# ibrahimhroob/SPS

Hardware: AMD Instinct MI355X
Metric: scans/sec @100k pts, 0.1 m voxel (higher is better)
Workload: dtype f32; 1 GPU; BASELINE config 2: single ~100k-pt LiDAR-like scan + variant-B submap, 0.1 m voxel, CustomMinkUNet14 fp32, 1 scan per step per GPU (4 distinct scans cycled); scan_points=100824, rows=153557, streams_per_gpu=8, compact_arenas=True

## Files before the change

### sps_amd/csrc/conv_kernels.inc.h

```cpp

typedef float floatx4 __attribute__((ext_vector_type(4)));

struct ConvArgs {
  const float *in;
  float *out;
  const float *Wu;
  const float *scale;
  const float *shift;
  const float *res;
  const int *nbr;
  const uint32_t *tmask;
  const int *n_out;
  const int *abort_flag;
  int out_rows;
  int64_t ldn;
  int ldi, ldo, ldr;
  int K, cin, cout, NT, upk;
  int relu, S;
  float inv_upk;
  float in_const;
  uint32_t in_bytes, wu_bytes, nbr_bytes;
  int tile_cap;
  int trace_on;
  const float *in2;
  int ldi2, upk2;
  uint32_t in2_bytes;
  const float *fin_w;
  float *fin_out;
  float fin_b;
  const uint32_t *rb_e;
  const unsigned char *rb_k;
  const int *rb_cnt;
  int rb_supertiles;
  const int4 *px_order;
  const int4 *tile_order;
  int order_ways;
  const float *up_Wu, *up_scale, *up_shift;
  const int *up_down;
  const uint32_t *up_tmask;
  float *up_out;
  int64_t up_ldn;
  int up_ldo, up_cout, up_rows;
  uint32_t up_wu_bytes;
};

#ifndef SPS_KCHUNK
#define SPS_KCHUNK 32
#endif
constexpr int KCHUNK = SPS_KCHUNK;
constexpr uint32_t OOR = 0xFFFF0000u;
typedef unsigned int u32x4 __attribute__((ext_vector_type(4)));

#if defined(SPS_WAVE_TRACE)
__device__ unsigned long long g_wave_trace[4 * 32768];
#endif

template <int NTW, int G, int MINW, bool DS, bool FIN, int S, int CG = 1, int UNT = 0, bool U4 = false>
__global__ __launch_bounds__((S == 8 ? 512 : 256) * CG, MINW) void k_conv(ConvArgs a) {
#if defined(SPS_WAVE_TRACE)
  const unsigned long long tr_t0 = wall_clock64();
  unsigned long long tr_t1 = 0;
  int tr_tiles = 0, tr_units = 0;
#endif
  static_assert(CG == 1 || (S == 4 && !FIN), "column groups share a workgroup only in the four-split geometry");
  static_assert(UNT == 0 || S == 4, "the fused transposed convolution needs one tile per workgroup");
  constexpr int NW1 = S == 8 ? 8 : 4;
  constexpr int NWV = NW1 * CG;
  __shared__ unsigned char klist[NWV][128];
  __shared__ uint32_t aoff_s[NWV][KCHUNK * 16];
  __shared__ uint32_t woff_s[NWV][KCHUNK];
  if (a.abort_flag && *a.abort_flag) return;
  const int count = *a.n_out;
  const int ntiles = (count + 15) >> 4;
  const int lane = threadIdx.x & 63, wave = __builtin_amdgcn_readfirstlane((int)(threadIdx.x >> 6));
  const int r = lane & 15, q = lane >> 4;
  const int cg = CG == 1 ? 0 : wave / NW1;
  const int w1 = CG == 1 ? wave : wave - cg * NW1;
  const int nt0 = ((int)blockIdx.x * CG + cg) * NTW;
  constexpr int tpw = NW1 / S;
  const int tl = S == 1 ? w1 : w1 / S;
  const int split = S == 1 ? 0 : w1 - tl * S;
  __shared__ float red_s[S > 1 ? CG * (NW1 - tpw) * NTW * 4 * 64 : 1];
  constexpr int XLD = CG * NTW * 16 + 4;
  __shared__ __attribute__((aligned(16))) float x_s[UNT > 0 ? 16 * XLD : 4];
  unsigned char *kl = klist[wave];
  uint32_t *ao = aoff_s[wave];
  uint32_t *wo = woff_s[wave];
  const __amdgpu_buffer_rsrc_t rsA = __builtin_amdgcn_make_buffer_rsrc((void *)a.in, 0, (int)a.in_bytes, 0x00020000);
  const __amdgpu_buffer_rsrc_t rsW = __builtin_amdgcn_make_buffer_rsrc((void *)a.Wu, 0, (int)a.wu_bytes, 0x00020000);
  const __amdgpu_buffer_rsrc_t rsN = __builtin_amdgcn_make_buffer_rsrc((void *)a.nbr, 0, (int)a.nbr_bytes, 0x00020000);
  const uint32_t ldn32 = (uint32_t)a.ldn;
  const int upk = a.upk;
  const uint32_t ldi4 = (uint32_t)a.ldi * 4u;
  const uint32_t wunit = (uint32_t)a.NT * 256u;
  const uint32_t wlane = (uint32_t)nt0 * 256u + (uint32_t)r * 16u;
  const int kstep = 4 / upk, cstep = 4 % upk;
  float esc[NTW], esh[NTW];
#pragma unroll
  for (int nt = 0; nt < NTW; ++nt) {
    const int col = (nt0 + nt) * 16 + r;
    esc[nt] = col < a.cout ? a.scale[col] : 0.f;
    esh[nt] = col < a.cout ? a.shift[col] : 0.f;
  }
  const float efw = (FIN && r < a.cout) ? a.fin_w[r] : 0.f;
  const int pos_first = blockIdx.y * tpw + tl;
  const int tile_first = a.tile_order ? -1 : pos_first;
  uint32_t pw0 = 0u, pw1 = 0u;
  if (a.tmask && tile_first >= 0 && tile_first < a.tile_cap) {
    pw0 = a.tmask[(size_t)tile_first * 4 + (lane >> 5)];
    pw1 = a.tmask[(size_t)tile_first * 4 + 2 + (lane >> 5)];
  }
  for (int grp = blockIdx.y; grp * tpw < ntiles; grp += gridDim.y) {
    const int pos = grp * tpw + tl;
    const bool active = pos < ntiles;
    int tile = pos;
    int4 oent = make_int4(0, 0, 0, 0);
    if (a.tile_order && active) {
      int idx = pos;
      if (a.order_ways > 0) idx = balanced_index(pos, ntiles, a.order_ways);
      oent = a.tile_order[idx];
      tile = oent.x;
    }
    if (S == 1 && !active) continue;
    const int row0 = tile * 16;
    int nk = 1;
    __builtin_amdgcn_wave_barrier();
    if (a.tmask) {
      uint32_t w0 = pw0, w1 = pw1;
      if (!active) {
        w0 = w1 = 0u;
      } else if (a.tile_order) {
        w0 = (lane >> 5) ? (uint32_t)oent.z : (uint32_t)oent.y;
        w1 = (lane >> 5) ? 0u : (uint32_t)oent.w;
      } else if (tile != tile_first) {
        const uint32_t *m = a.tmask + (size_t)tile * 4;
        w0 = m[lane >> 5];
        w1 = m[2 + (lane >> 5)];
      }
      const bool b0 = (w0 >> (lane & 31)) & 1u, b1 = lane < 32 && ((w1 >> (lane & 31)) & 1u);
      const unsigned long long bal0 = __ballot(b0), bal1 = __ballot(b1);
      const unsigned long long lt = (1ull << lane) - 1ull;
      const int n0 = __popcll(bal0);
      if (b0) kl[__popcll(bal0 & lt)] = (unsigned char)((lane >> 5) * 27 + (lane & 31));
      if (b1) kl[n0 + __popcll(bal1 & lt)] = (unsigned char)(54 + lane);
      nk = n0 + __popcll(bal1);
// ... 981 lines not shown
```

### sps_amd/csrc/map_kernels.inc.h

```cpp

enum NbrKind { NBR_3333 = 0, NBR_5551 = 1 };

typedef unsigned int u32x4 __attribute__((ext_vector_type(4)));

struct LevelView {
  const int *vblock;
  const unsigned char *vbit;
  const uint64_t *bkey;
  const unsigned long long *bmask;
  const int *bbase;
  const int *badj;
  const int *bparent;
  const int *bchild;
  const uint4 *bmb;
};

__device__ inline bool tile_mask_or(uint32_t *tmask, int u, int k, bool present) {
  const unsigned long long bal = __ballot(present);
  const int lane = threadIdx.x & 63;
  const bool any = ((bal >> (lane & 48)) & 0xFFFFull) != 0ull;
  if ((lane & 15) == 0 && any) atomicOr(&tmask[(size_t)(u >> 4) * 4 + (k >> 5)], 1u << (k & 31));
  return any;
}

struct MapsArgs {
  LevelView L[NLV];
  int *nbr3[NLV];
  uint32_t *tm3[NLV];
  int *down[NLV], *parent_row[NLV];
  uint32_t *tmdown[NLV];
  const int *counts;
  int chunk_off[NLV + 1];
  int64_t ldn[NLV];
  uint32_t *rb_e[NLV];
  unsigned char *rb_k[NLV];
  int *rb_cnt[NLV];
};

constexpr uint32_t PX_PAD = (1u << 30) | 64u;
static_assert(SPS_MAX_POINTS <= (1 << 23), "PX_PAD's input row 2^23 must lie beyond every feature buffer (row capacity <= SPS_MAX_POINTS)");
constexpr int PX_SEG_CH = 108;
constexpr int PX_CH_MAX = 324;
constexpr int PX_KSEG = 224;
constexpr int PX_KSTRIDE = 3 * PX_KSEG;
constexpr int PX_HALF_LEVELS = 1;
constexpr bool px_half_level(int l) { return (PX_HALF_LEVELS >> l) & 1; }
static_assert(PX_KSEG >= 2 * PX_SEG_CH && PX_KSEG % 4 == 0, "one offset byte per half-chunk");
constexpr int PX_LEVELS = 3;

__device__ inline int level_of_chunk(const MapsArgs &a, int first_level, int &local, int bid) {
  int l = first_level;
  while (l + 1 < NLV && bid >= a.chunk_off[l + 1]) ++l;
  local = bid - a.chunk_off[l];
  return l;
}

template <int R>
__device__ inline void lookup_run(const LevelView &L, int u, int dy, int dz, int dt, int k0, int *__restrict__ nbr,
                                  int64_t ldn, uint32_t *__restrict__ tmask) {
  const int r = L.vblock[u];
  const int bit = L.vbit[u];
  const int px = bit & 3, ty = ((bit >> 2) & 3) + dy, tz = (bit >> 4) + dz;
  const int ad0 = (dt + 1) * 27 + ((tz >> 2) + 1) * 9 + ((ty >> 2) + 1) * 3 + 1;
  const int nbit0 = ((tz & 3) << 4) | ((ty & 3) << 2);
  int last_bo = 99, base = 0;
  unsigned long long mk = 0ull;
#pragma unroll
  for (int dx = -R; dx <= R; ++dx) {
    const int tx = px + dx;
    const int bo = tx >> 2;
    if (bo != last_bo) {
      last_bo = bo;
      const int nb = L.badj[(size_t)r * 81 + ad0 + bo];
      mk = nb >= 0 ? L.bmask[nb] : 0ull;
      base = nb >= 0 ? L.bbase[nb] : 0;
    }
    const int nbit = nbit0 | (tx & 3);
    int row = -1;
    if ((mk >> nbit) & 1ull) row = base + __popcll(mk & ((1ull << nbit) - 1ull));
    const int k = k0 + dx + R;
    if (tile_mask_or(tmask, u, k, row >= 0)) nbr[(size_t)k * ldn + u] = row;
  }
}

template <bool TM, bool RB, int GR = 16>
__device__ inline void build_nbr3_t(const MapsArgs &a, int l, int local, int nchunks, int slice) {
  const int n = a.counts[l];
  const LevelView L = a.L[l];
  int *__restrict__ nbr = a.nbr3[l];
  uint32_t *__restrict__ tmask = a.tm3[l];
  const int64_t ldn = a.ldn[l];
  static_assert(GR == 16 || GR == 8, "rulebook padding granule: a chunk or a half-chunk");
  constexpr int GM = GR - 1, GS = GR == 16 ? 4 : 3;
  const int lane = threadIdx.x & 63;
  const int nround = (n + 63) & ~63;
  uint32_t *__restrict__ rbe = a.rb_e[l];
  unsigned char *__restrict__ rbk = a.rb_k[l];
  int *__restrict__ rbc = a.rb_cnt[l];
  const uint32_t tocc = reinterpret_cast<const uint32_t *>(a.counts)[TOCC];
  constexpr uint32_t OOR = 0xFFFFFFFFu;
  const __amdgpu_buffer_rsrc_t rsAdj = __builtin_amdgcn_make_buffer_rsrc((void *)L.badj, 0, (int)0xFFFFFFFEu, 0x00020000);
  const __amdgpu_buffer_rsrc_t rsBmb = __builtin_amdgcn_make_buffer_rsrc((void *)L.bmb, 0, (int)0xFFFFFFFEu, 0x00020000);
  for (int u = local * 256 + (int)threadIdx.x; u < nround; u += nchunks * 256) {
    const bool ok = u < n;
    const int r_raw = L.vblock[u];
    const int bit_raw = L.vbit[u];
    const int r = ok ? r_raw : 0;
    const int bit = ok ? bit_raw : 0;
    const int px = bit & 3, py = (bit >> 2) & 3, pz = bit >> 4;
    const int nt = ok ? (int)((L.bkey[r] >> 54) & 0x1F) + slice - 1 : -1;
    const bool act = nt >= 0 && nt < 32 && ((tocc >> nt) & 1u);
    if (!__any(act)) {
      if (TM && (lane & 15) == 0 && ok) tmask[(size_t)(u >> 4) * 4 + slice] = 0u;
      if (RB && lane == 0) rbc[(size_t)(u >> 6) * 4 + slice] = 0;
      continue;
    }
    const uint32_t adj4 = ((uint32_t)r * 81u + (uint32_t)slice * 27u) * 4u;
    const int sx = px == 0 ? -1 : (px == 3 ? 1 : 0), sy = py == 0 ? -1 : (py == 3 ? 1 : 0), sz = pz == 0 ? -1 : (pz == 3 ? 1 : 0);
    uint32_t mlo[8], mhi[8];
    int bs[8], nbv[8];
#pragma unroll
    for (int c = 0; c < 8; ++c) {
      const bool need = act && (!(c & 1) || sx != 0) && (!(c & 2) || sy != 0) && (!(c & 4) || sz != 0);
      const int e = (((c & 4) ? sz : 0) + 1) * 9 + (((c & 2) ? sy : 0) + 1) * 3 + (((c & 1) ? sx : 0) + 1);
      const int v = (int)__builtin_amdgcn_raw_buffer_load_b32(rsAdj, (need && !(SPS_ABLATE_FE & 32)) ? adj4 + (uint32_t)e * 4u : OOR, 0, 0);
      nbv[c] = need ? v : -1;
    }
#pragma unroll
    for (int c = 0; c < 8; ++c) {
      const u32x4 q = __builtin_amdgcn_raw_buffer_load_b128(rsBmb, (nbv[c] >= 0 && !(SPS_ABLATE_FE & 32)) ? (uint32_t)nbv[c] * 16u : OOR, 0, 0);
      mlo[c] = q.x, mhi[c] = q.y, bs[c] = (int)q.z;
      if constexpr (SPS_ABLATE_FE & 32) mlo[c] = 0x0F0F0F0Fu & (uint32_t)(nbv[c] + 1), mhi[c] = mlo[c];
    }
    bool oxv[3];
    uint32_t txl[3], txm[3];
#pragma unroll
    for (int d = 0; d < 3; ++d) {
      const int tx = px + d - 1;
      oxv[d] = (tx >> 2) != 0;
      txl[d] = (uint32_t)(tx & 3);
      txm[d] = (1u << txl[d]) - 1u;
    }
    uint32_t m = 0u;
    int cb = 0;
    uint32_t kinfo = 0u;
    uint32_t *__restrict__ eb = RB ? rbe + ((size_t)(u >> 6) * PX_CH_MAX + (size_t)slice * PX_SEG_CH) * 16 : nullptr;
    unsigned char *__restrict__ kb = RB ? rbk + (size_t)(u >> 6) * PX_KSTRIDE + slice * PX_KSEG : nullptr;
#pragma unroll 1
    for (int dz = -1; dz <= ((SPS_ABLATE_FE & 128) ? -2 : 1); ++dz) {
      const int tz = pz + dz;
      const bool oz = (tz >> 2) != 0;
      const bool half = (tz & 2) != 0;
      uint32_t zlo[4], zhi[4];
      int zb[4];
#pragma unroll
      for (int k = 0; k < 4; ++k) zlo[k] = oz ? mlo[k + 4] : mlo[k], zhi[k] = oz ? mhi[k + 4] : mhi[k], zb[k] = oz ? bs[k + 4] : bs[k];
#pragma unroll
      for (int dy = -1; dy <= 1; ++dy) {
        const int ty = py + dy;
        const bool oy = (ty >> 2) != 0;
        const uint32_t sh = (uint32_t)((((tz & 1) << 4) | ((ty & 3) << 2)));
        uint32_t nib[2];
        int pre[2];
#pragma unroll
        for (int k = 0; k < 2; ++k) {
// ... 16 lines not shown
            const bool any = ((bal >> (lane & 48)) & 0xFFFFull) != 0ull;
            if (any && ok && nbr && !(SPS_ABLATE_FE & 64)) nbr[(size_t)(27 * slice + j) * ldn + u] = row;
            m |= any ? 1u << j : 0u;
          }
          if constexpr (RB) {
            if (bal != 0ull) {
              const int cnt = __popcll(bal);
              const int below = (int)__builtin_amdgcn_mbcnt_hi((uint32_t)(bal >> 32), __builtin_amdgcn_mbcnt_lo((uint32_t)bal, 0u));
              const int pos = present ? below : cnt + lane - below;
              if ((present || pos < ((cnt + GM) & ~GM)) && !(SPS_ABLATE_FE & 64)) eb[cb * GR + pos] = present ? ((uint32_t)row << 7) | (uint32_t)lane : PX_PAD;
              const int ng = (cnt + GM) >> GS;
              kinfo = lane == j ? (uint32_t)cb | ((uint32_t)ng << 16) : kinfo;
              cb += ng;
            }
          }
        }
      }
    }
    if constexpr (RB) {
      const int first = (int)(kinfo & 0xFFFFu), ng = lane < 27 ? (int)(kinfo >> 16) : 0;
#pragma unroll
      for (int i = 0; i < 64 / GR; ++i)
        if (i < ng) kb[first + i] = (unsigned char)(27 * slice + lane);
      if constexpr (GR == 8) {
        if (cb & 1) {
          if (lane < 8 && !(SPS_ABLATE_FE & 64)) eb[cb * 8 + lane] = PX_PAD;
          if (ng > 0 && first + ng == cb) kb[cb] = (unsigned char)(27 * slice + lane);
        }
        cb = (cb + 1) >> 1;
      }
      if (lane == 0) rbc[(size_t)(u >> 6) * 4 + slice] = (SPS_ABLATE_FE & 64) ? 0 : cb;
    }
    if (TM && (lane & 15) == 0 && ok) tmask[(size_t)(u >> 4) * 4 + slice] = m;
  }
}

__device__ inline void build_nbr3(const MapsArgs &a, int bid, int slice) {
  int local;
  const int l = level_of_chunk(a, 0, local, bid);
  const int nchunks = a.chunk_off[l + 1] - a.chunk_off[l];
  const bool rb = a.rb_e[l] != nullptr, tm = a.nbr3[l] != nullptr || !rb;
  if (rb && px_half_level(l)) {
    if (tm) build_nbr3_t<true, true, 8>(a, l, local, nchunks, slice);
    else build_nbr3_t<false, true, 8>(a, l, local, nchunks, slice);
  }
  else if (rb && tm) build_nbr3_t<true, true>(a, l, local, nchunks, slice);
  else if (rb) build_nbr3_t<false, true>(a, l, local, nchunks, slice);
  else build_nbr3_t<true, false>(a, l, local, nchunks, slice);
}

__device__ inline bool tile_mask_test(const uint32_t *__restrict__ tmask, int u, int k, bool slice_words) {
  const int w = slice_words ? k / 27 : k >> 5, b = slice_words ? k - 27 * w : k & 31;
  return (tmask[(size_t)(u >> 4) * 4 + w] >> b) & 1u;
}

__global__ __launch_bounds__(256) void k_build_nbr5(const int *__restrict__ n_out, LevelView L, int *__restrict__ nbr,
                                                     int64_t ldn, uint32_t *__restrict__ tmask) {
  const int n = *n_out;
  const int c = blockIdx.y;
  const int dy = c % 5 - 2, dz = c / 5 - 2;
  for (int u = blockIdx.x * blockDim.x + threadIdx.x; u < n; u += gridDim.x * blockDim.x)
    lookup_run<2>(L, u, dy, dz, 0, 5 * c, nbr, ldn, tmask);
}

__device__ inline void build_stride_maps(const MapsArgs &a, int bid) {
  int local;
  const int f = level_of_chunk(a, 0, local, bid);
  if (f >= NLV - 1) return;
  const int c = f + 1;
  const int nchunks = a.chunk_off[f + 1] - a.chunk_off[f];
  const LevelView F = a.L[f], C = a.L[c];
  const int nf = a.counts[f], nc = a.counts[c];
  const int lane = threadIdx.x & 63;
  for (int v = local * 256 + (int)threadIdx.x; v < nf; v += nchunks * 256) {
    const int r = F.vblock[v];
    const int bit = F.vbit[v];
// ... 14 lines not shown
      const int r = C.vblock[u];
      const int bit = C.vbit[u];
      px = bit & 3, py = (bit >> 2) & 3, pz = bit >> 4;
      const int cb = C.bchild[(size_t)r * 8 + ((px >> 1) | ((py >> 1) << 1) | ((pz >> 1) << 2))];
      const u32x4 mb = __builtin_amdgcn_raw_buffer_load_b128(rsFmb, cb >= 0 ? (uint32_t)cb * 16u : 0xFFFFFFFFu, 0, 0);
      mk = ((unsigned long long)mb.y << 32) | mb.x;
      base = (int)mb.z;
    }
    uint32_t m = 0u;
#pragma unroll
    for (int k = 0; k < 8; ++k) {
      const int dx = k & 1, dy = (k >> 1) & 1, dz = (k >> 2) & 1;
      const int cbit = ((((pz & 1) << 1) + dz) << 4) | ((((py & 1) << 1) + dy) << 2) | (((px & 1) << 1) + dx);
      int row = -1;
      if ((mk >> cbit) & 1ull) row = base + __popcll(mk & ((1ull << cbit) - 1ull));
      if (ok) a.down[c][(size_t)k * a.ldn[c] + u] = row;
      const unsigned long long bal = __ballot(row >= 0);
      m |= ((bal >> (lane & 48)) & 0xFFFFull) != 0ull ? 1u << k : 0u;
    }
    if ((lane & 15) == 0 && ok) *reinterpret_cast<uint4 *>(a.tmdown[c] + (size_t)(u >> 4) * 4) = make_uint4(m, 0u, 0u, 0u);
  }
}

#if defined(SPS_FE_TRACE)
__device__ unsigned long long g_maps_trace[2 * 16384];
#endif
__global__ __launch_bounds__(256, 6) void k_maps(MapsArgs ma, int nchunk, int n_nbr) {
  if (ma.counts[ABORT]) return;
  const int bid = (int)blockIdx.x;
#if defined(SPS_FE_TRACE)
  if (threadIdx.x == 0 && bid < 16384) g_maps_trace[2 * bid] = wall_clock64();
#endif
  if (bid < n_nbr)
    build_nbr3(ma, bid % nchunk, bid / nchunk);
  else
    build_stride_maps(ma, bid - n_nbr);
#if defined(SPS_FE_TRACE)
  __syncthreads();
  if (threadIdx.x == 0 && bid < 16384) g_maps_trace[2 * bid + 1] = wall_clock64();
#endif
}

__global__ void k_count_pairs_rb(const uint32_t *__restrict__ rb_e, const unsigned char *__restrict__ rb_k,
                                 const int *__restrict__ rb_cnt, const int *__restrict__ n_ptr,
                                 unsigned long long *__restrict__ pairs, int half) {
  const int nst = (*n_ptr + 63) >> 6;
  const int64_t total = (int64_t)nst * 3 * PX_SEG_CH;
  for (int64_t i = (int64_t)blockIdx.x * blockDim.x + threadIdx.x; i < total; i += (int64_t)gridDim.x * blockDim.x) {
    const int st = (int)(i / (3 * PX_SEG_CH)), r = (int)(i - (int64_t)st * (3 * PX_SEG_CH));
    const int seg = r / PX_SEG_CH, lc = r - seg * PX_SEG_CH;
    if (lc >= rb_cnt[(size_t)st * 4 + seg]) continue;
    const uint32_t *e = rb_e + ((size_t)st * PX_CH_MAX + (size_t)seg * PX_SEG_CH + lc) * 16;
    const unsigned char *kb = rb_k + (size_t)st * PX_KSTRIDE + seg * PX_KSEG;
    int c0 = 0, c1 = 0;
    for (int j = 0; j < 8; ++j) c0 += e[j] != PX_PAD, c1 += e[8 + j] != PX_PAD;
    if (half) {
      if (c0) atomicAdd(&pairs[kb[2 * lc]], (unsigned long long)c0);
      if (c1) atomicAdd(&pairs[kb[2 * lc + 1]], (unsigned long long)c1);
    } else {
      atomicAdd(&pairs[kb[lc]], (unsigned long long)(c0 + c1));
    }
  }
}

__global__ void k_export_table(const int *__restrict__ nbr, int64_t ldn, int K, int slice_words, const int *__restrict__ n_ptr,
                               const uint32_t *__restrict__ tmask, int *__restrict__ out) {
  const int n = *n_ptr;
// ... 118 lines not shown
    const int w = __popc(m.x & 0x7FFFFFFu) + __popc(m.y & 0x7FFFFFFu) + __popc(m.z & 0x7FFFFFFu);
    sorted[start[w] + atomicAdd(&cursor[w], 1)] = make_int4(t, (int)m.x, (int)m.y, (int)m.z);
  }
}

constexpr int PX_ORDER_WAYS = 256;
__device__ inline void px_order_body(const TileOrderArgs &a, int l) {
  __shared__ int hist[PX_CH_MAX + 4], start[PX_CH_MAX + 4];
  if (a.counts[ABORT] || !a.rb_cnt[l]) return;
  const int nst = (a.counts[l] + 63) >> 6;
  const int *__restrict__ rbc = a.rb_cnt[l];
  for (int i = threadIdx.x; i < PX_CH_MAX + 4; i += blockDim.x) hist[i] = 0;
  __syncthreads();
  const int4 *__restrict__ rbc4 = reinterpret_cast<const int4 *>(rbc);
  for (int t = threadIdx.x; t < nst; t += blockDim.x) {
    const int4 ns = rbc4[t];
    atomicAdd(&hist[min(PX_CH_MAX, ns.x + ns.y + ns.z)], 1);
  }
  __syncthreads();
  bucket_starts_desc(hist, start, PX_CH_MAX + 1);
  __syncthreads();
  int *sorted = a.px_sorted[l];
  for (int t = threadIdx.x; t < nst; t += blockDim.x) {
    const int4 ns = rbc4[t];
    __hip_atomic_store(sorted + atomicAdd(&start[min(PX_CH_MAX, ns.x + ns.y + ns.z)], 1), t, __ATOMIC_RELAXED, __HIP_MEMORY_SCOPE_AGENT);
  }
  __syncthreads();
  for (int p = threadIdx.x; p < nst; p += blockDim.x) {
    const int st = __hip_atomic_load(sorted + balanced_index(p, nst, PX_ORDER_WAYS), __ATOMIC_RELAXED, __HIP_MEMORY_SCOPE_AGENT);
    const int4 ns = rbc4[st];
    a.px_order[l][p] = make_int4(st, ns.x, ns.y, ns.z);
  }
}
```

### sps_amd/csrc/sps_hip.hip

```cpp
#include <hip/hip_runtime.h>

#include <cmath>
#include <cstdarg>
#include <cstdint>
#include <cstdio>
#include <algorithm>
#include <array>
#include <cstdlib>
#include <cstring>
#include <map>
#include <memory>
#include <string>
#include <vector>

#include "../../include/sps_hip.h"

#if !defined(SPS_DIAG)
#undef SPS_ABLATE_A
#undef SPS_ABLATE_B
#undef SPS_ABLATE_HALF_B
#undef SPS_ABLATE_SKIP_B
#undef SPS_ABLATE_MFMA
#undef SPS_ABLATE_LOOP
#undef SPS_ABLATE_STAGE
// ... 181 lines not shown
  Level lv[SPS_NUM_LEVELS];
  SubmapScratch sub;
  bool tables_dirty = true;
  void *hash_keys_all = nullptr, *hash_mask_all = nullptr, *hash_first_all = nullptr, *hash_occ_all = nullptr;
  int *nbr5 = nullptr;
  int *counts = nullptr;
  int *err = nullptr;
  int *block_sums = nullptr;
  double *filter_part = nullptr;
  unsigned long long *scan_agg = nullptr;
  int *keep = nullptr;
  double *macc = nullptr;
  unsigned long long *pairs = nullptr;
  std::shared_ptr<sps_weights> weights;
  float *blob = nullptr;
  float *ss = nullptr;
  float *wu = nullptr;
  uint32_t *tm5 = nullptr;
  void *zero_region = nullptr;
  size_t zero_bytes = 0;
  float final_bias = 0.f;
  const NetSpec *net = nullptr;
  long long *vacc = nullptr;
  int *vcnt = nullptr;
  float *vfeat = nullptr;
  const float *cur_vfeat = nullptr;
  bool cur_head = false;
  bool diag_have_state = false;
  float *cat8 = nullptr, *b8t = nullptr, *b8o = nullptr, *logits = nullptr;
  float *x1 = nullptr, *b1t = nullptr, *cat7 = nullptr, *b7t = nullptr, *b7o = nullptr;
  float *x2 = nullptr, *b2t = nullptr, *cat6 = nullptr, *b6t = nullptr, *b6o = nullptr;
  float *x3 = nullptr, *b3t = nullptr, *cat5 = nullptr, *b5t = nullptr, *b5o = nullptr;
  float *x4 = nullptr, *b4t = nullptr, *b4o = nullptr;
  bool prof = false;
  std::vector<hipEvent_t> prof_ev;
  std::vector<std::string> prof_names;
  std::vector<std::string> prof_kernels;
  const char *last_kernel = "";
  size_t prof_n = 0;
  RadiusGrid rg{};
  std::vector<void *> rg_allocs;
  NdtMap ndt{};
  std::vector<void *> ndt_allocs;
  NdtDyn ndt_dyn{};
  NdtPyramid ndt_pyr{};
  std::vector<void *> ndt_pyr_allocs;
  int *item_counts = nullptr, *item_offsets = nullptr, *item_bsum = nullptr, *item_base = nullptr;
  int64_t item_cap = 0;
  HashTable map{};
  int64_t map_cap = 0;
  float map_ds = 0.f;
  void *map_keys_alloc = nullptr;
};

namespace {

int px_levels() {
  static const int m = [] { const char *e = diag_env("SPS_PX"); return (e ? atoi(e) : SPS_PX_DEFAULT) & ((1 << PX_LEVELS) - 1); }();
  return m;
}

int dev_alloc(sps_ctx *c, void **p, size_t bytes) {
  hipError_t e = hipMalloc(p, bytes ? bytes : 16);
  if (e != hipSuccess) return fail(SPS_ERR_NOMEM, "hipMalloc(%zu) failed: %s", bytes, hipGetErrorString(e));
  c->allocs.push_back(*p);
  return SPS_OK;
// ... 397 lines not shown
  a.wu_bytes = (uint32_t)(cs.wu_numel() * 4);
  a.nbr_bytes = (uint32_t)((size_t)cs.K * (size_t)c->capl[cc.level_out] * 4u);
  a.tile_cap = (int)(c->capl[cc.level_out] / 16);
  a.tile_order = (TILE_ORDER != 0 && cs.K == 81 && cc.level_out >= TILE_ORDER_FIRST_LEVEL) ? c->lv[cc.level_out].tile_order : nullptr;
  a.order_ways = TILE_ORDER == 2 ? TILE_ORDER_WAYS / std::max(1, a.NT / g.ntw) : 0;
  if (cc.up) {
    const ConvSpec &us = s.convs[s.find_conv(cc.up)];
    if (us.cin != cs.cout || cc.level_out < 1) return fail(SPS_ERR_INVALID, "%s cannot be fused into %s", cc.up, cc.name);
    a.up_Wu = c->wu + us.wu_off;
    a.up_scale = c->ss + us.ss_off;
    a.up_shift = c->ss + us.ss_off + us.cout;
    a.up_down = c->lv[cc.level_out].down;
    a.up_tmask = c->lv[cc.level_out].tmdown;
    a.up_ldn = c->capl[cc.level_out];
    a.up_out = cc.up_out;
    a.up_ldo = cc.up_ldo;
    a.up_cout = us.cout;
    a.up_rows = (int)c->capl[cc.level_out - 1];
    a.up_wu_bytes = (uint32_t)(us.wu_numel() * 4);
    grid.x = 1;
    a.order_ways = TILE_ORDER == 2 ? TILE_ORDER_WAYS : 0;
  }
  {
    static const char *trace_layer = diag_env("SPS_TRACE_LAYER");
    a.trace_on = trace_layer && std::strcmp(trace_layer, cc.name) == 0;
  }
  if (cs.cin == 1) {
    TileOrderArgs to{};
    const int g0 = grid_for(c->cap, 64, 4096);
    int gto = 0;
    if (TILE_ORDER != 0) {
      for (int l = 0; l < NLV; ++l) {
        const bool px = l < PX_LEVELS && ((px_levels() >> l) & 1) && c->lv[l].px_order;
        to.tm3[l] = (c->lv[l].nbr3 || !px) ? c->lv[l].tm3 : nullptr, to.order[l] = c->lv[l].tile_order;
        to.rb_cnt[l] = px ? c->lv[l].rb_cnt : nullptr, to.px_sorted[l] = c->lv[l].px_sorted, to.px_order[l] = c->lv[l].px_order;
      }
      to.counts = c->counts;
      gto = NLV - TILE_ORDER_FIRST_LEVEL + PX_LEVELS;
    }
    c->last_kernel = c->cur_vfeat ? "k_conv0_feat" : "k_conv0_fused";
    {
      static const int c0mode = [] { const char *e = diag_env("SPS_DIAG_CONV0"); return e ? atoi(e) : 0; }();
      if (c0mode == 1) {
        hipLaunchKernelGGL(k_conv0_fused, dim3((unsigned)gto), dim3(256), 0, st, a.n_out, c->lv[0].view(), c->blob + cs.w_off, a.scale,
                           a.shift, a.in_const, a.out, a.ldo, 1, to, 0);
        return SPS_OK;
      }
      if (c0mode == 2) gto = 0;
    }
    if (c->cur_vfeat) {
      hipLaunchKernelGGL(k_conv0_feat, dim3((unsigned)(g0 + gto)), dim3(256), 0, st, a.n_out,
                         c->lv[0].view(), c->blob + cs.w_off, a.scale, a.shift, c->cur_vfeat, a.out, a.ldo, to, g0);
      return SPS_OK;
    }
    hipLaunchKernelGGL(k_conv0_fused, dim3((unsigned)(g0 + gto)), dim3(256), 0, st, a.n_out,
                       c->lv[0].view(), c->blob + cs.w_off, a.scale, a.shift, a.in_const, a.out, a.ldo, 1, to, g0);
    return SPS_OK;
  }
  if (cs.K == 8 && std::strncmp(cc.name, "convtr", 6) == 0) {
    {
      const int coarse = cc.level_out + 1;
      a.nbr = c->lv[coarse].down;
      a.tmask = c->lv[coarse].tmdown;
      a.n_out = c->counts + coarse;
      a.ldn = c->capl[coarse];
      a.tile_cap = (int)(c->capl[coarse] / 16);
      a.out_rows = (int)c->capl[cc.level_out];
      int64_t gu = (c->cap / 16) >> coarse;
      if (gu < 64) gu = 64;
      if (gu > 8192) gu = 8192;
      const dim3 gr((unsigned)gu);
      c->last_kernel = "k_upconv";
      if (a.NT == 1)
        hipLaunchKernelGGL((k_upconv<1>), gr, dim3(256), 0, st, a);
      else if (a.NT == 2)
        hipLaunchKernelGGL((k_upconv<2>), gr, dim3(256), 0, st, a);
      else
        hipLaunchKernelGGL((k_upconv<4>), gr, dim3(256), 0, st, a);
      return SPS_OK;
    }
  }
  const bool ds = cs.ds_cin > 0;
  if (cc.level_out < PX_LEVELS && ((px_levels() >> cc.level_out) & 1) && c->lv[cc.level_out].rb_e && cs.K == 81 && a.NT == 1 && (cs.cout == 8 || cs.cout == 16) &&
      (cs.cin == 8 || cs.cin == 16 || cs.cin == 24) && (!cc.fin || cs.cout == 8)) {
    int64_t gs = (c->cap / 64) >> cc.level_out;
    if (gs < 64) gs = 64;
    if (gs > 4096) gs = 4096;
    const dim3 gridp((unsigned)gs);
    a.rb_e = c->lv[cc.level_out].rb_e;
    a.rb_k = c->lv[cc.level_out].rb_k;
    a.rb_cnt = c->lv[cc.level_out].rb_cnt;
// ... 17 lines not shown
      case 811: SPS_PX_LAUNCH(8, true, true, false); break;
      case 812: SPS_PX_LAUNCH(8, true, true, true); break;
      case 1601:
        if (cc.up) {
          if (cc.level_out != 1 || a.up_cout > 16) return fail(SPS_ERR_INVALID, "%s cannot be fused into %s", cc.up, cc.name);
          launch_px<SPS_PX1, 16, false, true, false, SPS_PX1_W, true>(gridp, st, a);
        } else {
          SPS_PX_LAUNCH(16, false, true, false);
        }
        break;
      case 1610: SPS_PX_LAUNCH(16, true, false, false); break;
      case 2400: SPS_PX_LAUNCH(24, false, false, false); break;
      default: return fail(SPS_ERR_INVALID, "no k_conv_px instantiation for %s", cc.name);
    }
#undef SPS_PX_LAUNCH
    return SPS_OK;
  }
  if (cs.K == 81 && !a.nbr)
    return fail(SPS_ERR_INVALID, "%s has no pair-exact instantiation and the inference-only context keeps no neighbour table at level %d",
                cc.name, cc.level_out);
  if (cc.fin && !(g.ntw == 1 && ds && g.S == 1)) return fail(SPS_ERR_INVALID, "final fusion needs NT = 1, S = 1");
  c->last_kernel = cs.K == 81 ? (cc.level_out >= 2 ? "k_conv<3x3x3x3, levels 2-4>" : "k_conv<3x3x3x3, levels 0-1>") : "k_conv<2x2x2x1 stride 2>";
  if (cc.fin) {
    hipLaunchKernelGGL((k_conv<1, SPS_G1DS, SPS_W1, true, true, 1>), grid, dim3(256), 0, st, a);
    return SPS_OK;
  }
  unsigned lds_pad = 0;
#if defined(SPS_DIAG)
  {
    static const int pad = [] { const char *e = diag_env("SPS_CONV_LDS_PAD"); return e ? atoi(e) : 0; }();
    if (cc.level_out >= 2 && cs.K == 81) lds_pad = (unsigned)pad;
  }
#endif
  return launch_k_conv(a, g, ds, grid, st, lds_pad);
}

void permute_weights(const ConvSpec &cs, const float *W, float *Wu, const float *colscale = nullptr) {
  if (cs.cin == 1) {
    for (int k = 0; k < cs.K; ++k)
      for (int n = 0; n < 16; ++n) Wu[k * 16 + n] = n < cs.cout ? W[(size_t)k * cs.cout + n] : 0.f;
    return;
  }
  const int upk = cs.upk(), NT = cs.nt();
  for (int k = 0; k < cs.K; ++k)
    for (int c4 = 0; c4 < upk; ++c4) {
      const int u = k * upk + c4;
      for (int nt = 0; nt < NT; ++nt)
        for (int n = 0; n < 16; ++n)
          for (int sidx = 0; sidx < 4; ++sidx) {
            const int col = nt * 16 + n;
            float v = col < cs.cout ? W[((size_t)k * cs.cin + 4 * c4 + sidx) * cs.cout + col] : 0.f;
            if (colscale && col < cs.cout) v *= colscale[col];
            Wu[(((size_t)u * NT + nt) * 16 + n) * 4 + sidx] = v;
          }
    }
}

void prof_mark(sps_ctx *c, const char *name, hipStream_t st) {
  if (!c->prof) return;
  if (c->prof_n >= c->prof_ev.size()) {
    hipEvent_t e;
    if (hipEventCreate(&e) != hipSuccess) return;
    c->prof_ev.push_back(e);
    c->prof_names.emplace_back();
    c->prof_kernels.emplace_back();
  }
// ... 397 lines not shown
    int co[NLV + 1] = {0};
    for (int i = 0; i < NLV; ++i) co[i + 1] = co[i] + grid_for(((cap >> 3) >> (2 * (NLV - 1 - i))) * 27, 256, 2048);
#if defined(SPS_FE_TRACE)
    g_link_geom[0] = gb;
    for (int l = 0; l <= NLV; ++l) g_link_geom[1 + l] = co[l];
#endif
    if (no_merge & 2) {
      hipLaunchKernelGGL(k_link_adj, dim3(4 * gb), dim3(256), 0, st, pa, gb, co[1], co[2], co[3], co[4], co[5]);
      hipLaunchKernelGGL(k_link_adj, dim3(co[NLV]), dim3(256), 0, st, pa, 0, co[1], co[2], co[3], co[4], co[5]);
    } else {
      hipLaunchKernelGGL(k_link_adj, dim3(4 * gb + co[NLV]), dim3(256), 0, st, pa, gb, co[1], co[2], co[3], co[4], co[5]);
    }
  }
  c->last_kernel = "k_link_adj";
  prof_mark(c, "pyramid", st);
  MapsArgs ma{};
  int off = 0;
  for (int l = 0; l < NLV; ++l) {
    const Level &L = c->lv[l];
    ma.L[l] = L.view();
    ma.nbr3[l] = L.nbr3;
    ma.tm3[l] = L.tm3;
    ma.down[l] = L.down;
    ma.parent_row[l] = L.inv;
    ma.tmdown[l] = L.tmdown;
    ma.chunk_off[l] = off;
    off += grid_for(cap >> l, 256, 1024);
  }
  ma.chunk_off[NLV] = off;
  ma.counts = c->counts;
  for (int l = 0; l < PX_LEVELS; ++l)
    if (((px_levels() >> l) & 1) && !fo.front_only) ma.rb_e[l] = c->lv[l].rb_e, ma.rb_k[l] = c->lv[l].rb_k, ma.rb_cnt[l] = c->lv[l].rb_cnt;
  for (int l = 0; l < NLV; ++l) ma.ldn[l] = c->capl[l];
#if defined(SPS_FE_TRACE)
  g_maps_geom[0] = off;
  for (int l = 0; l <= NLV; ++l) g_maps_geom[1 + l] = ma.chunk_off[l];
#endif
  if (no_merge & 4) {
    hipLaunchKernelGGL(k_maps, dim3(off * 3), dim3(256), 0, st, ma, off, off * 3);
    hipLaunchKernelGGL(k_maps, dim3(ma.chunk_off[NLV - 1]), dim3(256), 0, st, ma, off, 0);
  } else {
    hipLaunchKernelGGL(k_maps, dim3(off * 3 + ma.chunk_off[NLV - 1]), dim3(256), 0, st, ma, off, off * 3);
  }
  c->diag_have_state = true;
  }
  c->last_kernel = "k_maps";
  prof_mark(c, "maps", st);
  if (fo.front_only) {
    HIP_TRY(hipGetLastError());
    return SPS_OK;
  }
  Level *lv = c->lv;
  c->cur_vfeat = fo.feats ? c->vfeat : nullptr;
  const bool fuse_final = !fo.head;
  const ConvCall calls[] = {
      {"conv0p1s1", nullptr, 1, c->cat8 + 8, 16, Map{c->nbr5, c->tm5}, 0, nullptr, 0, 1},
      {"conv1p1s2", c->cat8 + 8, 16, c->x1, 8, Map{lv[1].down, lv[1].tmdown}, 1, nullptr, 0, 1},
      {"block1.0.conv1", c->x1, 8, c->b1t, 8, Map{lv[1].nbr3, lv[1].tm3}, 1, nullptr, 0, 1},
      {"block1.0.conv2", c->b1t, 8, c->cat7 + 16, 24, Map{lv[1].nbr3, lv[1].tm3}, 1, c->x1, 8, 1},
      {"conv2p2s2", c->cat7 + 16, 24, c->x2, 8, Map{lv[2].down, lv[2].tmdown}, 2, nullptr, 0, 1},
      {"block2.0.conv1", c->x2, 8, c->b2t, 16, Map{lv[2].nbr3, lv[2].tm3}, 2, nullptr, 0, 1},
      {"block2.0.conv2", c->b2t, 16, c->cat6 + 32, 48, Map{lv[2].nbr3, lv[2].tm3}, 2, nullptr, 0, 1, c->x2, 8},
      {"conv3p4s2", c->cat6 + 32, 48, c->x3, 16, Map{lv[3].down, lv[3].tmdown}, 3, nullptr, 0, 1},
      {"block3.0.conv1", c->x3, 16, c->b3t, 32, Map{lv[3].nbr3, lv[3].tm3}, 3, nullptr, 0, 1},
      {"block3.0.conv2", c->b3t, 32, c->cat5 + 64, 96, Map{lv[3].nbr3, lv[3].tm3}, 3, nullptr, 0, 1, c->x3, 16},
      {"conv4p8s2", c->cat5 + 64, 96, c->x4, 32, Map{lv[4].down, lv[4].tmdown}, 4, nullptr, 0, 1},
      {"block4.0.conv1", c->x4, 32, c->b4t, 64, Map{lv[4].nbr3, lv[4].tm3}, 4, nullptr, 0, 1},
      {"block4.0.conv2", c->b4t, 64, c->b4o, 64, Map{lv[4].nbr3, lv[4].tm3}, 4, nullptr, 0, 1, c->x4, 32, false,
       (FUSE_UP & 1) ? "convtr4p16s2" : nullptr, c->cat5, 96},
      {"convtr4p16s2", c->b4o, 64, c->cat5, 96, Map{lv[4].down, lv[4].tmdown}, 3, nullptr, 0, 1},
      {"block5.0.conv1", c->cat5, 96, c->b5t, 64, Map{lv[3].nbr3, lv[3].tm3}, 3, nullptr, 0, 1},
      {"block5.0.conv2", c->b5t, 64, c->b5o, 64, Map{lv[3].nbr3, lv[3].tm3}, 3, nullptr, 0, 1, c->cat5, 96, false,
       (FUSE_UP & 2) ? "convtr5p8s2" : nullptr, c->cat6, 48},
      {"convtr5p8s2", c->b5o, 64, c->cat6, 48, Map{lv[3].down, lv[3].tmdown}, 2, nullptr, 0, 1},
      {"block6.0.conv1", c->cat6, 48, c->b6t, 32, Map{lv[2].nbr3, lv[2].tm3}, 2, nullptr, 0, 1},
      {"block6.0.conv2", c->b6t, 32, c->b6o, 32, Map{lv[2].nbr3, lv[2].tm3}, 2, nullptr, 0, 1, c->cat6, 48, false,
       (FUSE_UP & 4) ? "convtr6p4s2" : nullptr, c->cat7, 24},
      {"convtr6p4s2", c->b6o, 32, c->cat7, 24, Map{lv[2].down, lv[2].tmdown}, 1, nullptr, 0, 1},
      {"block7.0.conv1", c->cat7, 24, c->b7t, 16, Map{lv[1].nbr3, lv[1].tm3}, 1, nullptr, 0, 1},
      {"block7.0.conv2", c->b7t, 16, c->b7o, 16, Map{lv[1].nbr3, lv[1].tm3}, 1, nullptr, 0, 1, c->cat7, 24, false,
       (FUSE_UP & 8) ? "convtr7p2s2" : nullptr, c->cat8, 16},
      {"convtr7p2s2", c->b7o, 16, c->cat8, 16, Map{lv[1].down, lv[1].tmdown}, 0, nullptr, 0, 1},
      {"block8.0.conv1", c->cat8, 16, c->b8t, 8, Map{lv[0].nbr3, lv[0].tm3}, 0, nullptr, 0, 1},
      {"block8.0.conv2", c->b8t, 8, c->b8o, 8, Map{lv[0].nbr3, lv[0].tm3}, 0, nullptr, 0, 1, c->cat8, 16, fuse_final},
  };
  const char *fused_up = nullptr;
  static const char *const fused_stage[][2] = {{"block4.0.conv2", "block4.0.conv2+convtr4p16s2"},
                                               {"block5.0.conv2", "block5.0.conv2+convtr5p8s2"},
                                               {"block6.0.conv2", "block6.0.conv2+convtr6p4s2"},
                                               {"block7.0.conv2", "block7.0.conv2+convtr7p2s2"}};
  static const int skip_class = [] { const char *e = diag_env("SPS_DIAG_SKIP_CLASS"); return e ? atoi(e) : 0; }();
  for (const ConvCall &cc : calls) {
    if (skip_convs) break;
    if (skip_class) {
      const bool tr = std::strncmp(cc.name, "convtr", 6) == 0, c0 = std::strcmp(cc.name, "conv0p1s1") == 0;
      const bool blk = std::strncmp(cc.name, "block", 5) == 0, strided = !tr && !c0 && !blk;
      const int cls = blk ? (cc.level_out >= 2 ? 1 : 2) : strided ? 4 : tr ? 8 : 16;
      if (skip_class & cls) continue;
    }
    if (fused_up && std::strcmp(cc.name, fused_up) == 0) {
      fused_up = nullptr;
      continue;
    }
    int rc = run_conv(c, cc, st);
    if (rc != SPS_OK) return rc;
    const char *stage = cc.name;
    if (cc.up) {
      fused_up = cc.up;
      for (const auto &fs : fused_stage)
        if (std::strcmp(cc.name, fs[0]) == 0) stage = fs[1];
    }
    prof_mark(c, stage, st);
  }
  c->cur_vfeat = nullptr;
  const int gs = (int)((n + 255) / 256), gbc = grid_for(cap >> 2, 256, 256);
  if (fo.head) {
    const NetSpec &s = *c->net;
    const ConvSpec &fs = s.convs[s.find_conv("final")];
    hipLaunchKernelGGL(k_slice_head, dim3((unsigned)gs), dim3(256), 0, st, c->b8o, 8, L0.inv, (int)n,
                       c->blob + fs.w_off, c->blob + s.bias_off, s.out_channels, fo.act, scores, fo.ldo, c->counts + 15,
                       fo.n_dev);
    c->last_kernel = "k_slice_head";
    prof_mark(c, "slice_head", st);
    if (!skip_front) hipLaunchKernelGGL(k_bhash_cleanup, dim3(gbc * NLV), dim3(256), 0, st, pa, gbc);
  } else if (skip_front || (no_merge & 8)) {
    hipLaunchKernelGGL(k_slice_sigmoid, dim3((unsigned)gs), dim3(256), 0, st, c->logits, L0.inv, (int)n, scores, c->counts + 15);
    if (!skip_front) hipLaunchKernelGGL(k_bhash_cleanup, dim3(gbc * NLV), dim3(256), 0, st, pa, gbc);
    if (fo.metrics_out) {
      HIP_TRY(hipMemsetAsync(fo.metrics_out, 0, (size_t)fo.n_batches * 8 * sizeof(double), st));
      hipLaunchKernelGGL(k_metrics, dim3((unsigned)grid_for(n, 1024, 128)), dim3(256), 0, st, scores, (int)n,
                         MetricsArgs{coords, ld, fo.eps, fo.n_batches, fo.metrics_out});
    }
  } else {
    const MetricsArgs mt{coords, ld, fo.eps, fo.n_batches, fo.metrics_out};
    const int gst = fo.metrics_out ? grid_for(n, 1024, 256) : gs;
    hipLaunchKernelGGL(k_tail, dim3((unsigned)(gst + gbc * NLV)), dim3(256), 0, st, c->logits, L0.inv, (int)n, scores, gst,
                       pa, gbc, mt);
  }
  c->last_kernel = fo.head ? "k_bhash_cleanup" : "k_tail";
// ... 724 lines not shown
```

Measured before the change: 4083 scans/s.

## Fuse conv0 into the neighbour-map kernel and fold tile ordering into the next conv

Computes the first 5x5x5 convolution (constant input, 8 outputs) inside the level-0 neighbour-map builder, reusing the occupancy bitmasks it already loads to build per-row presence words and feed MFMA directly. This removes the separate conv0 launch and its reading of the neighbour table. The tile/px ordering work that conv0 used to host is deferred and either run as extra workgroups prepended to the first eligible k_conv launch or as a standalone k_orders kernel. The trade-off is more register and LDS pressure in the maps kernel, and a reordering of slices so that the conv0-carrying slice runs first.

Result: faster. 4127 scans/s, median of 6 (+1.1%).

```diff
diff --git a/sps_amd/csrc/conv_kernels.inc.h b/sps_amd/csrc/conv_kernels.inc.h
--- a/sps_amd/csrc/conv_kernels.inc.h
+++ b/sps_amd/csrc/conv_kernels.inc.h
@@ -42,6 +42,8 @@
   int64_t up_ldn;
   int up_ldo, up_cout, up_rows;
   uint32_t up_wu_bytes;
+  TileOrderArgs ord;
+  int ord_wg;
 };
 
 #ifndef SPS_KCHUNK
@@ -55,8 +57,20 @@
 __device__ unsigned long long g_wave_trace[4 * 32768];
 #endif
 
-template <int NTW, int G, int MINW, bool DS, bool FIN, int S, int CG = 1, int UNT = 0, bool U4 = false>
+template <int NTW, int G, int MINW, bool DS, bool FIN, int S, int CG = 1, int UNT = 0, bool U4 = false, bool ORD = false>
 __global__ __launch_bounds__((S == 8 ? 512 : 256) * CG, MINW) void k_conv(ConvArgs a) {
+  if constexpr (ORD) {
+    static_assert(S == 1 && CG == 1 && UNT == 0, "the hosting launch has one column group: blockIdx.y counts workgroups");
+    if ((int)blockIdx.y < a.ord_wg) {
+      const int which = (int)blockIdx.y;
+      if (which < NLV - TILE_ORDER_FIRST_LEVEL)
+        tile_order_body(a.ord, which);
+      else
+        px_order_body(a.ord, which - (NLV - TILE_ORDER_FIRST_LEVEL));
+      return;
+    }
+  }
+  const int by = ORD ? (int)blockIdx.y - a.ord_wg : (int)blockIdx.y, gy = ORD ? (int)gridDim.y - a.ord_wg : (int)gridDim.y;
 #if defined(SPS_WAVE_TRACE)
   const unsigned long long tr_t0 = wall_clock64();
   unsigned long long tr_t1 = 0;
@@ -103,14 +117,14 @@
     esh[nt] = col < a.cout ? a.shift[col] : 0.f;
   }
   const float efw = (FIN && r < a.cout) ? a.fin_w[r] : 0.f;
-  const int pos_first = blockIdx.y * tpw + tl;
+  const int pos_first = by * tpw + tl;
   const int tile_first = a.tile_order ? -1 : pos_first;
   uint32_t pw0 = 0u, pw1 = 0u;
   if (a.tmask && tile_first >= 0 && tile_first < a.tile_cap) {
     pw0 = a.tmask[(size_t)tile_first * 4 + (lane >> 5)];
     pw1 = a.tmask[(size_t)tile_first * 4 + 2 + (lane >> 5)];
   }
-  for (int grp = blockIdx.y; grp * tpw < ntiles; grp += gridDim.y) {
+  for (int grp = by; grp * tpw < ntiles; grp += gy) {
     const int pos = grp * tpw + tl;
     const bool active = pos < ntiles;
     int tile = pos;
diff --git a/sps_amd/csrc/map_kernels.inc.h b/sps_amd/csrc/map_kernels.inc.h
--- a/sps_amd/csrc/map_kernels.inc.h
+++ b/sps_amd/csrc/map_kernels.inc.h
@@ -2,6 +2,7 @@
 enum NbrKind { NBR_3333 = 0, NBR_5551 = 1 };
 
 typedef unsigned int u32x4 __attribute__((ext_vector_type(4)));
+typedef float floatx4 __attribute__((ext_vector_type(4)));
 
 struct LevelView {
   const int *vblock;
@@ -35,6 +36,10 @@
   uint32_t *rb_e[NLV];
   unsigned char *rb_k[NLV];
   int *rb_cnt[NLV];
+  const float *c0_w, *c0_scale, *c0_shift;
+  float *c0_out;
+  int c0_ldo;
+  float c0_in;
 };
 
 constexpr uint32_t PX_PAD = (1u << 30) | 64u;
@@ -83,8 +88,9 @@
   }
 }
 
-template <bool TM, bool RB, int GR = 16>
+template <bool TM, bool RB, int GR = 16, bool C0 = false>
 __device__ inline void build_nbr3_t(const MapsArgs &a, int l, int local, int nchunks, int slice) {
+  __shared__ uint4 c0_pw[C0 ? 256 : 1];
   const int n = a.counts[l];
   const LevelView L = a.L[l];
   int *__restrict__ nbr = a.nbr3[l];
@@ -110,13 +116,14 @@
     const int px = bit & 3, py = (bit >> 2) & 3, pz = bit >> 4;
     const int nt = ok ? (int)((L.bkey[r] >> 54) & 0x1F) + slice - 1 : -1;
     const bool act = nt >= 0 && nt < 32 && ((tocc >> nt) & 1u);
-    if (!__any(act)) {
+    if (!C0 && !__any(act)) {
       if (TM && (lane & 15) == 0 && ok) tmask[(size_t)(u >> 4) * 4 + slice] = 0u;
       if (RB && lane == 0) rbc[(size_t)(u >> 6) * 4 + slice] = 0;
       continue;
     }
     const uint32_t adj4 = ((uint32_t)r * 81u + (uint32_t)slice * 27u) * 4u;
-    const int sx = px == 0 ? -1 : (px == 3 ? 1 : 0), sy = py == 0 ? -1 : (py == 3 ? 1 : 0), sz = pz == 0 ? -1 : (pz == 3 ? 1 : 0);
+    const int sx = C0 ? (px < 2 ? -1 : 1) : px == 0 ? -1 : (px == 3 ? 1 : 0), sy = C0 ? (py < 2 ? -1 : 1) : py == 0 ? -1 : (py == 3 ? 1 : 0),
+              sz = C0 ? (pz < 2 ? -1 : 1) : pz == 0 ? -1 : (pz == 3 ? 1 : 0);
     uint32_t mlo[8], mhi[8];
     int bs[8], nbv[8];
 #pragma unroll
@@ -131,6 +138,35 @@
       const u32x4 q = __builtin_amdgcn_raw_buffer_load_b128(rsBmb, (nbv[c] >= 0 && !(SPS_ABLATE_FE & 32)) ? (uint32_t)nbv[c] * 16u : OOR, 0, 0);
       mlo[c] = q.x, mhi[c] = q.y, bs[c] = (int)q.z;
       if constexpr (SPS_ABLATE_FE & 32) mlo[c] = 0x0F0F0F0Fu & (uint32_t)(nbv[c] + 1), mhi[c] = mlo[c];
+    }
+    if constexpr (C0) {
+      const bool xneg = px < 2;
+      const uint32_t xs = (uint32_t)(px - 2 + (xneg ? 4 : 0));
+      uint32_t bm[4] = {0u, 0u, 0u, 0u};
+#pragma unroll
+      for (int dz = -2; dz <= 2; ++dz) {
+        const int tz = pz + dz;
+        const bool oz = (tz >> 2) != 0, half = (tz & 2) != 0;
+        uint32_t wl[2], wh[2];
+#pragma unroll
+        for (int k = 0; k < 2; ++k) {
+          const uint32_t own = half ? (oz ? mhi[4 + 2 * k] : mhi[2 * k]) : (oz ? mlo[4 + 2 * k] : mlo[2 * k]);
+          const uint32_t oth = half ? (oz ? mhi[5 + 2 * k] : mhi[1 + 2 * k]) : (oz ? mlo[5 + 2 * k] : mlo[1 + 2 * k]);
+          wl[k] = xneg ? oth : own, wh[k] = xneg ? own : oth;
+        }
+#pragma unroll
+        for (int dy = -2; dy <= 2; ++dy) {
+          const int ty = py + dy;
+          const bool oy = (ty >> 2) != 0;
+          const uint32_t sh = (uint32_t)(((tz & 1) << 4) | ((ty & 3) << 2));
+          const uint32_t n0 = ((oy ? wl[1] : wl[0]) >> sh) & 0xFu, n1 = ((oy ? wh[1] : wh[0]) >> sh) & 0xFu;
+          const uint32_t pres = ((n0 | (n1 << 4)) >> xs) & 0x1Fu;
+          const int b = 5 * ((dy + 2) + 5 * (dz + 2));
+          bm[b >> 5] |= pres << (b & 31);
+          if ((b & 31) > 27) bm[(b >> 5) + 1] |= pres >> (32 - (b & 31));
+        }
+      }
+      c0_pw[u & 255] = make_uint4(bm[0], bm[1], bm[2], bm[3]);
     }
     bool oxv[3];
     uint32_t txl[3], txm[3];
@@ -213,16 +249,66 @@
       if (lane == 0) rbc[(size_t)(u >> 6) * 4 + slice] = (SPS_ABLATE_FE & 64) ? 0 : cb;
     }
     if (TM && (lane & 15) == 0 && ok) tmask[(size_t)(u >> 4) * 4 + slice] = m;
-  }
-}
+    if constexpr (C0) {
+      int ln = lane;
+      asm volatile("" : "+v"(ln));
+      const int r = ln & 15, q = ln >> 4;
+      const float esc = a.c0_scale[r & 7], esh = a.c0_shift[r & 7];
+      const __amdgpu_buffer_rsrc_t rsW = __builtin_amdgcn_make_buffer_rsrc((void *)a.c0_w, 0, 125 * 8 * 4, 0x00020000);
+      const uint32_t cbits = __float_as_uint(a.c0_in);
+      const int row0 = u - ln;
+      __builtin_amdgcn_wave_barrier();
+      floatx4 acc[4];
+#pragma unroll
+      for (int t = 0; t < 4; ++t) acc[t] = floatx4{0.f, 0.f, 0.f, 0.f};
+      const uint32_t *pw = reinterpret_cast<const uint32_t *>(c0_pw + ((row0 & 255) + r));
+#pragma unroll 1
+      for (int w = 0; w < 4; ++w) {
+        uint32_t bq[4];
+#pragma unroll
+        for (int t = 0; t < 4; ++t) bq[t] = pw[64 * t + w] >> q;
+        const uint32_t wk = r < 8 ? (uint32_t)((32 * w + q) * 8 + r) * 4u : 0x80000000u;
+#pragma unroll
+        for (int g = 0; g < 8; ++g) {
+          const float bv = __uint_as_float(__builtin_amdgcn_raw_buffer_load_b32(rsW, wk + 128u * g, 0, 0));
+#pragma unroll
+          for (int t = 0; t < 4; ++t) {
+            const float av = __uint_as_float((uint32_t)__builtin_amdgcn_sbfe((int)bq[t], 4 * g, 1) & cbits);
+            acc[t] = __builtin_amdgcn_mfma_f32_16x16x4f32(av, bv, acc[t], 0, 0, 0);
+          }
+        }
+      }
+      if (r < 8) {
+#pragma unroll
+        for (int t = 0; t < 4; ++t)
+#pragma unroll
+          for (int i = 0; i < 4; ++i) {
+            const int ro = row0 + 16 * t + q * 4 + i;
+            if (ro < n) {
+              const float y = acc[t][i] * esc + esh;
+              a.c0_out[(size_t)ro * a.c0_ldo + r] = fmaxf(y, 0.f);
+            }
+          }
+      }
+      __builtin_amdgcn_wave_barrier();
+    }
+  }
+}
+
+__host__ __device__ constexpr bool level_has_tile_masks(bool has_nbr_table, bool has_rulebook) { return has_nbr_table || !has_rulebook; }
 
 __device__ inline void build_nbr3(const MapsArgs &a, int bid, int slice) {
   int local;
   const int l = level_of_chunk(a, 0, local, bid);
   const int nchunks = a.chunk_off[l + 1] - a.chunk_off[l];
-  const bool rb = a.rb_e[l] != nullptr, tm = a.nbr3[l] != nullptr || !rb;
+  const bool rb = a.rb_e[l] != nullptr, tm = level_has_tile_masks(a.nbr3[l] != nullptr, rb);
   if (rb && px_half_level(l)) {
-    if (tm) build_nbr3_t<true, true, 8>(a, l, local, nchunks, slice);
+    static_assert(PX_HALF_LEVELS == 1, "conv0 rides in the 8-pair instantiation: level 0 alone");
+    if (a.c0_out && slice == 1) {
+      if (tm) build_nbr3_t<true, true, 8, true>(a, 0, local, nchunks, 1);
+      else build_nbr3_t<false, true, 8, true>(a, 0, local, nchunks, 1);
+    }
+    else if (tm) build_nbr3_t<true, true, 8>(a, l, local, nchunks, slice);
     else build_nbr3_t<false, true, 8>(a, l, local, nchunks, slice);
   }
   else if (rb && tm) build_nbr3_t<true, true>(a, l, local, nchunks, slice);
@@ -303,7 +389,10 @@
   if (threadIdx.x == 0 && bid < 16384) g_maps_trace[2 * bid] = wall_clock64();
 #endif
   if (bid < n_nbr)
-    build_nbr3(ma, bid % nchunk, bid / nchunk);
+    {
+      const int b3 = bid / nchunk;
+      build_nbr3(ma, bid % nchunk, ma.c0_out ? (b3 == 0 ? 1 : b3 == 1 ? 0 : 2) : b3);
+    }
   else
     build_stride_maps(ma, bid - n_nbr);
 #if defined(SPS_FE_TRACE)
@@ -488,3 +577,11 @@
     a.px_order[l][p] = make_int4(st, ns.x, ns.y, ns.z);
   }
 }
+
+__global__ __launch_bounds__(256) void k_orders(TileOrderArgs to) {
+  const int which = (int)blockIdx.x;
+  if (which < NLV - TILE_ORDER_FIRST_LEVEL)
+    tile_order_body(to, which);
+  else
+    px_order_body(to, which - (NLV - TILE_ORDER_FIRST_LEVEL));
+}
diff --git a/sps_amd/csrc/sps_hip.hip b/sps_amd/csrc/sps_hip.hip
--- a/sps_amd/csrc/sps_hip.hip
+++ b/sps_amd/csrc/sps_hip.hip
@@ -237,6 +237,10 @@
   float *x2 = nullptr, *b2t = nullptr, *cat6 = nullptr, *b6t = nullptr, *b6o = nullptr;
   float *x3 = nullptr, *b3t = nullptr, *cat5 = nullptr, *b5t = nullptr, *b5o = nullptr;
   float *x4 = nullptr, *b4t = nullptr, *b4o = nullptr;
+  bool conv0_in_maps = false;
+  bool ord_pending = false;
+  TileOrderArgs ord_args{};
+  int ord_wg = 0;
   bool prof = false;
   std::vector<hipEvent_t> prof_ev;
   std::vector<std::string> prof_names;
@@ -700,11 +704,15 @@
     if (TILE_ORDER != 0) {
       for (int l = 0; l < NLV; ++l) {
         const bool px = l < PX_LEVELS && ((px_levels() >> l) & 1) && c->lv[l].px_order;
-        to.tm3[l] = (c->lv[l].nbr3 || !px) ? c->lv[l].tm3 : nullptr, to.order[l] = c->lv[l].tile_order;
+        to.tm3[l] = level_has_tile_masks(c->lv[l].nbr3 != nullptr, px) ? c->lv[l].tm3 : nullptr, to.order[l] = c->lv[l].tile_order;
         to.rb_cnt[l] = px ? c->lv[l].rb_cnt : nullptr, to.px_sorted[l] = c->lv[l].px_sorted, to.px_order[l] = c->lv[l].px_order;
       }
       to.counts = c->counts;
       gto = NLV - TILE_ORDER_FIRST_LEVEL + PX_LEVELS;
+    }
+    if (c->conv0_in_maps) {
+      c->ord_pending = gto > 0, c->ord_args = to, c->ord_wg = gto;
+      return SPS_OK;
     }
     c->last_kernel = c->cur_vfeat ? "k_conv0_feat" : "k_conv0_fused";
     {
@@ -725,6 +733,10 @@
                        c->lv[0].view(), c->blob + cs.w_off, a.scale, a.shift, a.in_const, a.out, a.ldo, 1, to, g0);
     return SPS_OK;
   }
+  const bool host_orders = c->ord_pending && cs.K == 8 && !is_up && cc.level_out == 1 && g.ntw == 1 && g.S == 1 && grid.x == 1 &&
+                           cs.ds_cin == 0 && !cc.fin && !cc.up;
+  if (c->ord_pending && !host_orders) hipLaunchKernelGGL(k_orders, dim3((unsigned)c->ord_wg), dim3(256), 0, st, c->ord_args);
+  c->ord_pending = false;
   if (cs.K == 8 && std::strncmp(cc.name, "convtr", 6) == 0) {
     {
       const int coarse = cc.level_out + 1;
@@ -808,6 +820,12 @@
     if (cc.level_out >= 2 && cs.K == 81) lds_pad = (unsigned)pad;
   }
 #endif
+  if (host_orders) {
+    a.ord = c->ord_args, a.ord_wg = c->ord_wg;
+    grid.y += (unsigned)a.ord_wg;
+    hipLaunchKernelGGL((k_conv<1, SPS_G1, SPS_W1, false, false, 1, 1, 0, false, true>), grid, dim3(256), lds_pad, st, a);
+    return SPS_OK;
+  }
   return launch_k_conv(a, g, ds, grid, st, lds_pad);
 }
 
@@ -1271,6 +1289,18 @@
   for (int l = 0; l < PX_LEVELS; ++l)
     if (((px_levels() >> l) & 1) && !fo.front_only) ma.rb_e[l] = c->lv[l].rb_e, ma.rb_k[l] = c->lv[l].rb_k, ma.rb_cnt[l] = c->lv[l].rb_cnt;
   for (int l = 0; l < NLV; ++l) ma.ldn[l] = c->capl[l];
+  static const bool c0_apart = [] { const char *e = diag_env("SPS_DIAG_CONV0"); return e && atoi(e) != 0; }();
+  c->conv0_in_maps = ma.rb_e[0] && px_half_level(0) && !fo.feats && !fo.front_only && !c0_apart && !(no_merge & 4);
+  if (c->conv0_in_maps) {
+    const NetSpec &s = *c->net;
+    const ConvSpec &c0 = s.convs[s.find_conv("conv0p1s1")];
+    ma.c0_w = c->blob + c0.w_off;
+    ma.c0_scale = c->ss + c0.ss_off;
+    ma.c0_shift = c->ss + c0.ss_off + c0.cout;
+    ma.c0_out = c->cat8 + 8;
+    ma.c0_ldo = 16;
+    ma.c0_in = 0.5f;
+  }
 #if defined(SPS_FE_TRACE)
   g_maps_geom[0] = off;
   for (int l = 0; l <= NLV; ++l) g_maps_geom[1 + l] = ma.chunk_off[l];
@@ -1283,8 +1313,10 @@
   }
   c->diag_have_state = true;
   }
+  if (skip_front) c->conv0_in_maps = false;
+  c->ord_pending = false;
   c->last_kernel = "k_maps";
-  prof_mark(c, "maps", st);
+  prof_mark(c, c->conv0_in_maps ? "maps+conv0p1s1" : "maps", st);
   if (fo.front_only) {
     HIP_TRY(hipGetLastError());
     return SPS_OK;
@@ -1344,6 +1376,7 @@
     int rc = run_conv(c, cc, st);
     if (rc != SPS_OK) return rc;
     const char *stage = cc.name;
+    if (c->conv0_in_maps && std::strcmp(cc.name, "conv0p1s1") == 0) continue;
     if (cc.up) {
       fused_up = cc.up;
       for (const auto &fs : fused_stage)
```
